# nicrie/xmca

Hardware: AMD Instinct MI355X
Metric: MCA solve+rotate throughput (ms_per_step = solve+rotate wall-clock, ms); rule_n surrogates/s in `rule_n` (higher is better)
Workload: dtype f64; 1 GPU; C2: synthetic EOF T=2920 x N=10000 float64 (generator A), solve() + rotate(n_rot=10, power=1); parallelism=replicas x1 (solve/rotate do not shard); rule_n run-sharded x1

## Files before the change

### xmca_amd/csrc/jacobi.h

```cpp
#pragma once
#include <algorithm>
#include <cmath>
#include <cstring>

#include "common.h"
#include "gemm.h"
#include "cholesky.h"
#include "tridiag.h"
#include "tridiag_vec.h"
#include "jacobi_kernels.h"

namespace xmca {

struct EvdInfo {
  int sweeps = 0;
  int tile = 0;
  int slots = 0;
  double last_off = 0.0;
  int lr_step = 0;
  double diag_spread = 0;
  int tridiag = 0;
  int n_eigvec = 0;
};

// ... 279 lines not shown
                          std::vector<double>& lam_host, double* lam_dev, double* Zr, double* Zi, int64_t ldz,
                          EvdInfo* info = nullptr, bool nearly_diagonal = false, int n_lead = -1, TrdLeadHook* lead_hook = nullptr) {
  const bool cplx = Ai != nullptr;
  const bool part = Zr && n_lead >= 0 && n_lead < n;
  if (part) XMCA_CHECK(n_lead >= 1, XMCA_ERR_INVALID, "hermitian_evd: n_lead must be at least 1 when vectors are wanted");
  DevBuf<double> full[2];
  double *Fr = Zr, *Fi = Zi;
  int64_t ldf = ldz;
  auto all_rows = [&] {
    if (!part || Fr != Zr) return;
    Fr = full[0].ensure((size_t)n * n);
    Fi = cplx ? full[1].ensure((size_t)n * n) : nullptr;
    ldf = n;
  };
  auto hand_out = [&] {
    if (!part) return;
    const size_t row = sizeof(double) * (size_t)n;
    XMCA_HIP(hipMemcpy2DAsync(Zr, sizeof(double) * (size_t)ldz, Fr, row, row, (size_t)n_lead, hipMemcpyDeviceToDevice, st));
    if (cplx) XMCA_HIP(hipMemcpy2DAsync(Zi, sizeof(double) * (size_t)ldz, Fi, row, row, (size_t)n_lead, hipMemcpyDeviceToDevice, st));
    XMCA_HIP(hipStreamSynchronize(st));
  };
  const int trd_min_n = [] { const char* e = std::getenv("XMCA_TRIDIAG_MIN_N"); return e ? std::atoi(e) : 192; }();
  if (!Zr && !nearly_diagonal && trd_enabled() && n >= trd_min_n && trd_fits(n, Ai != nullptr)) {
    TrdParams P = trd_reduce(st, ws.trd, Ar, Ai, n, lda, false);
    if (xmca_trace("trdsum")) trd_trace_checksums(st, P, Ar, n, lda);
    trd_eigenvalues(st, ws.trd, P, lam_host, lam_dev, ws.lam_tmp);
    if (info) {
      *info = EvdInfo{};
      info->tridiag = 1;
    }
    return;
  }
  if (Zr && !nearly_diagonal && evd_vectors_by_reduction(n, Ai != nullptr)) {
    ws.trdv.count_call();
    TrdParams P = trd_reduce(st, ws.trd, Ar, Ai, n, lda, true);
    trd_wy_prepare(st, ws.trdv, ws.gws, P, Ai != nullptr);
    std::vector<double> lam_t;
    trd_eigenvalues(st, ws.trd, P, lam_t, lam_dev, ws.lam_tmp, ws.trdv.lam_asc.ensure((size_t)n));
    if (part) {
      const int kp = trd_partial_count(lam_t, n, n_lead);
      bool ran = false, done = false;
      const bool rep_lead = trd_repeated_leading(lam_t, n, kp);
      if (kp < n && !rep_lead) {
        ran = true;
        done = trd_eigenvectors_partial(st, ws.trdv, ws.gws, P, cplx, kp, n_lead, Zr, Zi, ldz);
      }
      if (xmca_trace("solve"))
        std::fprintf(stderr, "xmca: eigh n = %d, %d leading vectors wanted: %d formed%s\n", n, n_lead, done ? kp : n,
                     done ? "" : (kp >= n ? " (no gap within the cap)" : rep_lead ? " (repeated eigenvalues)" : " (clean-up refused)"));
      if (done) {
        XMCA_HIP(hipStreamSynchronize(st));
        lam_host = lam_t;
        if (info) {
          *info = EvdInfo{};
          info->tridiag = 1;
          info->n_eigvec = kp;
        }
        return;
      }
      if (ran) ws.trdv.prepared = true;
    }
    bool repeated = false;
    {
      const double lmax = n > 0 ? std::max(std::fabs(lam_t.front()), std::fabs(lam_t.back())) : 0.0;
      for (int i = 0; i + 1 < n && !repeated; ++i) repeated = lam_t[(size_t)i] - lam_t[(size_t)i + 1] <= 2.2e-16 * lmax;
      if (repeated && xmca_trace("solve")) std::fprintf(stderr, "xmca: eigh n = %d: repeated eigenvalues - block Jacobi instead of twisted vectors\n", n);
    }
    if (repeated) {
      if (ws.trdv.prepared && !ws.trdv.joined && ws.trdv.side) XMCA_HIP(hipStreamSynchronize(ws.trdv.side));
      ws.trdv.prepared = false;
      ws.trdv.joined = true;
    }
    if (!repeated) all_rows();
    if (!repeated && trd_eigenvectors(st, ws.trd, ws.trdv, ws.gws, P, Ai != nullptr, Fr, Fi, ldf, part ? nullptr : lead_hook)) {
      XMCA_HIP(hipStreamSynchronize(st));
      lam_host = lam_t;
      if (info) {
        *info = EvdInfo{};
        info->tridiag = 1;
        info->n_eigvec = n;
      }
      hand_out();
      return;
    }
  }
  const double tol = Zr ? 1e-10 : 1e-8;
  all_rows();
  if (Ai) jacobi_evd<true, 32>(st, ws, Ar, Ai, n, lda, lam_host, lam_dev, Fr, Fi, ldf, tol, info);
  else if (n > 32) jacobi_evd<false, 64>(st, ws, Ar, nullptr, n, lda, lam_host, lam_dev, Fr, nullptr, ldf, tol, info);
  else jacobi_evd<false, 32>(st, ws, Ar, nullptr, n, lda, lam_host, lam_dev, Fr, nullptr, ldf, tol, info);
  hand_out();
}

}
// ... 1 lines not shown
```

### xmca_amd/csrc/tridiag.h

```cpp
#pragma once
#include <algorithm>
#include <cmath>
#include <cstring>
#include <vector>

#include "common.h"

namespace xmca {

constexpr int TRD_THREADS = 512;
constexpr int TRD_ROWS = 4;
constexpr int TRD_MAX_WGS = 256;
constexpr int TRD_MAX_ITERS = 32;

struct TrdParams {
  double* Ar;
  double* Ai;
  int64_t ld;
  int n;
  double* vb[2][2];
  double* pb[2][2];
  double* gp[2][2];
  double* tau[2];
  double* d;
  double* e;
  double* Vr;
// ... 900 lines not shown
    if (CPLX) { double* t1 = bV[1]; bV[1] = bX[1]; bX[1] = t1; }
    tpr = tr_next;
    tpi = ti_next;
    spr = sr_next;
    spi = si_next;
  }
}

__global__ void trd_prefill_kernel(const double* __restrict__ Wr, const double* __restrict__ Wi, int n, double* __restrict__ xch) {
  const int k = blockIdx.x * blockDim.x + threadIdx.x;
  if (k >= n) return;
  if (Wi) {
    xch[2 * k] = trd_untagged(Wr[k]);
    xch[2 * k + 1] = trd_untagged(Wi[k]);
  } else {
    xch[2 * k] = trd_untagged(Wr[k]);
  }
}

__global__ __launch_bounds__(256) void trd_maxabs_kernel(const double* __restrict__ Ar, const double* __restrict__ Ai, int n, int64_t lda,
                                                         unsigned long long* __restrict__ acc) {
  double m = 0.0;
  bool bad = false;
  for (int r = blockIdx.x; r < n; r += gridDim.x)
    for (int c = threadIdx.x; c < n; c += 256) {
      const double a = fabs(Ar[(int64_t)r * lda + c]), b = Ai ? fabs(Ai[(int64_t)r * lda + c]) : 0.0;
      if (!(a <= 1.7e308) || !(b <= 1.7e308)) bad = true;
      m = fmax(m, fmax(a, b));
    }
  for (int o = 32; o > 0; o >>= 1) m = fmax(m, __shfl_xor(m, o));
  if (__any(bad)) { if ((threadIdx.x & 63) == 0) atomicOr(acc + 1, 1ull); }
  else if ((threadIdx.x & 63) == 0 && m > 0.0) atomicMax(acc, (unsigned long long)__double_as_longlong(m));
}
__global__ void trd_scale_kernel(const unsigned long long* __restrict__ acc, double* __restrict__ scal) {
  const double g = __longlong_as_double((long long)acc[0]);
  const bool nan = acc[1] != 0ull;
  double f = 1.0;
  if (g > 0.0 && !nan) {
    int ex;
    frexp(g, &ex);
    f = ldexp(1.0, -ex);
  }
  scal[0] = f;
  scal[1] = nan ? 1.0 : 0.0;
}

__global__ void trd_copy_kernel(const double* __restrict__ Ar, const double* __restrict__ Ai, int n, int64_t lda, double* Wr, double* Wi,
                                int64_t ld, const double* __restrict__ scal) {
  const double f = scal[0];
  const int r = blockIdx.x;
  for (int c = threadIdx.x; c < ld; c += blockDim.x) {
    const bool in = c < n;
    Wr[(int64_t)r * ld + c] = in ? f * Ar[(int64_t)r * lda + c] : 0.0;
    if (Wi) Wi[(int64_t)r * ld + c] = in ? f * Ai[(int64_t)r * lda + c] : 0.0;
  }
}

constexpr int TRD_BIS_THREADS = 256;
__global__ __launch_bounds__(TRD_BIS_THREADS) void trd_bisect_kernel(const double* __restrict__ d, const double* __restrict__ e, int n,
                                                                   const double* __restrict__ scal, double* lam_desc, double* lam_asc_scaled, int* flag) {
  extern __shared__ __attribute__((aligned(16))) double bis_lds[];
  __shared__ double red[2][TRD_BIS_THREADS / 64];
  double* sd = bis_lds;
  double* se2 = bis_lds + n;
  const int tid = threadIdx.x;
  double gl = 1.7e308, gu = -1.7e308;
  bool bad = false;
// ... 74 lines not shown
  if (live && l == 0) {
    lam_desc[n - 1 - k] = 0.5 * (lo + hi) / scal[0];
    if (lam_asc_scaled) lam_asc_scaled[k] = 0.5 * (lo + hi);
  }
}

struct TrdWorkspace {
  DevBuf<double> W[2];
  DevBuf<double> V[2];
  DevBuf<double> vec;
  DevBuf<double> scal;
  DevBuf<int> flag;
  DevBuf<unsigned long long> prof;
  DevBuf<double> sync;
  DevBuf<unsigned int> flags;
  int resident_used = 0;
  int stages_used = 0;
  std::string last_desc;
  hipEvent_t ev[2] = {nullptr, nullptr};
  bool ev_pending = false;
  double reduce_ms = 0.0;
  long long reduce_calls = 0;
  long long resident_calls = 0;
  void ev_begin(hipStream_t st) {
    if (!ev[0]) { XMCA_HIP(hipEventCreate(&ev[0])); XMCA_HIP(hipEventCreate(&ev[1])); }
    XMCA_HIP(hipEventRecord(ev[0], st));
  }
  void ev_end(hipStream_t st) { XMCA_HIP(hipEventRecord(ev[1], st)); ev_pending = true; }
  void ev_collect() {
    if (!ev_pending) return;
    float t = 0.f;
    if (hipEventSynchronize(ev[1]) == hipSuccess && hipEventElapsedTime(&t, ev[0], ev[1]) == hipSuccess) { reduce_ms += t; ++reduce_calls; }
    ev_pending = false;
  }
  ~TrdWorkspace() { if (ev[0]) { (void)hipEventDestroy(ev[0]); (void)hipEventDestroy(ev[1]); } }
  double ms = 0.0;
};

inline bool trd_enabled() {
  const char* e = std::getenv("XMCA_TRIDIAG");
  return !(e && e[0] == '0');
}

inline size_t trd_step_lds(int n, bool cplx) { return (size_t)(((n + 3) + 1) & ~1) * 3 * (cplx ? 2 : 1) * sizeof(double); }

inline bool trd_fits(int n, bool cplx) {
// ... 84 lines not shown
      for (int cnc = nc - 4; cnc >= 4; cnc -= 4) {
        const int cap = cnc * 128;
        if (n <= cap) continue;
        const int c = ((n - cap + 255) / 256) * 256;
        if (c < n - 256 && (cuts.empty() || c > cuts.back())) cuts.push_back(c);
      }
    }
  }
  int begin = 0;
  for (size_t q = 0; q <= cuts.size(); ++q) {
    const int end = q < cuts.size() ? cuts[q] : n;
    TrdStage sg{};
    sg.col0 = begin;
    sg.nc = (q == 0 && !chain) ? nc : trd_stage_nc(n - begin, cplx);
    sg.rr = (q > 0 && chain && trd_pack_lanes()) ? trd_stage_rr_packed(sg.nc, cplx) : trd_stage_rr(sg.nc, cplx);
    sg.j_begin = begin;
    sg.j_end = end;
    st.push_back(sg);
    begin = end;
  }
  return st;
}

inline TrdParams trd_reduce(hipStream_t st, TrdWorkspace& ws, const double* Ar, const double* Ai, int n, int64_t lda, bool keep_reflectors) {
  const bool cplx = Ai != nullptr;
  const int nc = trd_resident_nc(n, cplx);
  const std::vector<TrdStage> stages = trd_plan(n, cplx, nc);
  int64_t ld = std::max<int64_t>(((int64_t)n + 2 + 15) & ~(int64_t)15, (int64_t)nc * 128);
  for (const TrdStage& sg : stages) ld = std::max<int64_t>(ld, (int64_t)sg.col0 + (int64_t)sg.nc * 128);
  const size_t nv = (size_t)((n + 8 + 15) & ~15);
  ws.W[0].ensure((size_t)n * ld);
  if (cplx) ws.W[1].ensure((size_t)n * ld);
  if (keep_reflectors) {
    ws.V[0].ensure((size_t)n * ld);
    XMCA_HIP(hipMemsetAsync(ws.V[0].get(), 0, sizeof(double) * (size_t)n * ld, st));
    if (cplx) {
      ws.V[1].ensure((size_t)n * ld);
      XMCA_HIP(hipMemsetAsync(ws.V[1].get(), 0, sizeof(double) * (size_t)n * ld, st));
    }
  }
  ws.vec.ensure(TrdLayout::doubles(nv));
  ws.scal.ensure(4);
  ws.flag.ensure(4);
  XMCA_HIP(hipMemsetAsync(ws.vec.get(), 0, sizeof(double) * TrdLayout::doubles(nv), st));
  XMCA_HIP(hipMemsetAsync(ws.flag.get(), 0, sizeof(int) * 4, st));
  TrdLayout lay{n, ld, nv, ws.vec.get()};
  TrdParams P = lay.params(ws.W[0].get(), cplx ? ws.W[1].get() : nullptr, keep_reflectors ? ws.V[0].get() : nullptr,
                           (keep_reflectors && cplx) ? ws.V[1].get() : nullptr);
  {
    unsigned long long* acc = reinterpret_cast<unsigned long long*>(ws.scal.get() + 2);
    XMCA_HIP(hipMemsetAsync(acc, 0, 2 * sizeof(unsigned long long), st));
    hipLaunchKernelGGL(trd_maxabs_kernel, dim3(std::min(n, 1024)), dim3(256), 0, st, Ar, Ai, n, lda, acc);
    hipLaunchKernelGGL(trd_scale_kernel, dim3(1), dim3(1), 0, st, acc, ws.scal.get());
  }
  hipLaunchKernelGGL(trd_copy_kernel, dim3(n), dim3(256), 0, st, Ar, Ai, n, lda, P.Ar, P.Ai, ld, ws.scal.get());
  ws.resident_used = 0;

  if (nc > 0) {
    PersistGate& gate = persist_gate();
    const int n_cus = gate.n_cus;
    const size_t lv = (size_t)(ld > (int64_t)nc * 128 ? ld : (int64_t)nc * 128);
    const size_t rec = cplx ? 4 : 2;
    const size_t sync_doubles = 2 * lv + 8 + 2 * rec * lv;
    ws.sync.ensure(sync_doubles);
    ws.flags.ensure(4);
    XMCA_HIP(hipMemsetAsync(ws.sync.get(), 0, sizeof(double) * sync_doubles, st));
    XMCA_HIP(hipMemsetAsync(ws.flags.get(), 0, sizeof(unsigned int) * 4, st));
    TrdSync S{};
    double* q = ws.sync.get();
    for (int c = 0; c < 2; ++c) { S.hand_u[c] = q; q += lv; }
    S.hand_s = q; q += 8;
    S.xch = q;
    S.xch_pb = (int)(rec * lv * sizeof(double));
    S.contiguous = in_surrogate_lanes() ? 1 : 0;
    S.spin_limit = trd_spin_limit();
    hipLaunchKernelGGL(trd_prefill_kernel, dim3(ceil_div(n, 256)), dim3(256), 0, st, P.Ar, P.Ai, n, S.xch);
    S.give_up = reinterpret_cast<int*>(ws.flags.get());
    using ResFn = void (*)(TrdParams, TrdSync, int);
    auto pick = [&](int snc, int srr) -> ResFn {
      if (cplx) {
        switch (snc) {
          case 4: return srr == 2 ? trd_resident_kernel<true, 4, 2> : trd_resident_kernel<true, 4, 1>;
          case 8: return srr == 2 ? trd_resident_kernel<true, 8, 2> : trd_resident_kernel<true, 8, 1>;
          case 12: return srr == 3 ? trd_resident_kernel<true, 12, 3> : trd_resident_kernel<true, 12, 2>;
          case 16: return trd_resident_kernel<true, 16, 2>;
          default: return trd_resident_kernel<true, 20, 2>;
        }
      }
      switch (snc) {
        case 4: return trd_resident_kernel<false, 4, 1>;
        case 8: return trd_resident_kernel<false, 8, 1>;
        case 12: return trd_resident_kernel<false, 12, 2>;
        case 16: return trd_resident_kernel<false, 16, 2>;
        case 20: return trd_resident_kernel<false, 20, 3>;
        default: return trd_resident_kernel<false, 24, 3>;
      }
    };
    static const char* prof_file_r = std::getenv("XMCA_TRD_PROF");
    if (prof_file_r) {
      P.prof = ws.prof.ensure((size_t)8 * n);
      XMCA_HIP(hipMemsetAsync(P.prof, 0, sizeof(unsigned long long) * 8 * (size_t)n, st));
    }
    int gave_up = 0;
    {
      PersistGate::Claim claim(gate, n_cus);
      ws.ev_begin(st);
      for (size_t q = 0; q < stages.size(); ++q) {
        const TrdStage& sg = stages[q];
        const int c0 = sg.col0, ns = n - c0;
        const int64_t off = (int64_t)c0 * ld + c0;
        TrdParams Pq = P;
        Pq.n = ns;
        Pq.Ar = P.Ar + off;
        if (P.Ai) Pq.Ai = P.Ai + off;
        Pq.d = P.d + c0; Pq.e = P.e + c0;
        Pq.tau[0] = P.tau[0] + c0; Pq.tau[1] = P.tau[1] + c0;
        if (P.Vr) Pq.Vr = P.Vr + off;
        if (P.Vi) Pq.Vi = P.Vi + off;
        if (P.prof) Pq.prof = P.prof + (size_t)8 * c0;
        TrdSync Sq = S;
        Sq.hand_u[0] = S.hand_u[0] + c0; Sq.hand_u[1] = S.hand_u[1] + c0;
        Sq.xch = S.xch + 2 * (size_t)c0;
        Sq.j_begin = sg.j_begin - c0;
        Sq.j_end = sg.j_end - c0;
        Sq.cont = q > 0 ? 1 : 0;
        const int wgs = std::max(1, std::min(std::min(n_cus, TRD_MAX_WGS), ceil_div(ns, (TRD_RES_THREADS / 64) * sg.rr)));
        const int first_res = std::max(0, ns - wgs * (TRD_RES_THREADS / 64) * sg.rr);
        const size_t lds = (size_t)sg.nc * 128 * 3 * (cplx ? 2 : 1) * sizeof(double);
        ResFn fn = pick(sg.nc, sg.rr);
        XMCA_HIP(hipFuncSetAttribute(reinterpret_cast<const void*>(fn), hipFuncAttributeMaxDynamicSharedMemorySize, 150 * 1024));
        hipLaunchKernelGGL(fn, dim3(wgs), dim3(TRD_RES_THREADS), lds, st, Pq, Sq, first_res);
      }
      ws.ev_end(st);
      XMCA_HIP(hipGetLastError());
      int dbg[4] = {0};
      XMCA_HIP(hipMemcpyAsync(dbg, S.give_up, sizeof(dbg), hipMemcpyDeviceToHost, st));
      XMCA_HIP(hipStreamSynchronize(st));
      gave_up = dbg[0];
      if (gave_up && xmca_trace("giveup"))
        std::fprintf(stderr, "xmca: trd_resident_kernel: workgroup %d ran out of its spins at column %d of its launch (n = %d, %d launches)\n", dbg[3], dbg[2], n, (int)stages.size());
    }
    ws.stages_used = (int)stages.size();
    {
      std::string d = stages.size() > 1 ? "chain of " + std::to_string(stages.size()) + " persistent launches: " : "";
      for (size_t q = 0; q < stages.size(); ++q) {
        const TrdStage& sg = stages[q];
        d += (q ? " -> " : "") + std::string("trd_resident_kernel<") + (cplx ? "complex" : "real") + ",NC=" + std::to_string(sg.nc) + ",RR=" + std::to_string(sg.rr) +
             ",tagged> columns [" + std::to_string(sg.j_begin) + "," + std::to_string(sg.j_end) + ")";
      }
      ws.last_desc = d;
    }
    if (prof_file_r) {
      std::vector<unsigned long long> hp((size_t)8 * n);
      XMCA_HIP(hipMemcpy(hp.data(), P.prof, sizeof(unsigned long long) * hp.size(), hipMemcpyDeviceToHost));
      if (FILE* f = std::fopen(prof_file_r, "w")) {
        for (int j = 0; j < n; ++j) {
          for (int q = 0; q < 7; ++q) std::fprintf(f, "%llu ", hp[(size_t)8 * j + q] - (q ? hp[(size_t)8 * j] : (j ? hp[(size_t)8 * (j - 1)] : hp[0])));
          std::fprintf(f, "\n");
        }
        std::fclose(f);
      }
      P.prof = nullptr;
    }
    if (!gave_up) {
      ws.resident_used = 1;
      ++ws.resident_calls;
      ws.ev_collect();
      return P;
    }
    ws.ev_pending = false;
    ws.resident_used = 2;
    ++persist_giveups();
    if (xmca_trace("giveup")) std::fprintf(stderr, "xmca: trd_resident_kernel (n = %d) gave up - repeated with one launch per column\n", n);
    hipLaunchKernelGGL(trd_copy_kernel, dim3(n), dim3(256), 0, st, Ar, Ai, n, lda, P.Ar, P.Ai, ld, ws.scal.get());
    XMCA_HIP(hipMemsetAsync(ws.vec.get(), 0, sizeof(double) * TrdLayout::doubles(nv), st));
    if (keep_reflectors) {
      XMCA_HIP(hipMemsetAsync(ws.V[0].get(), 0, sizeof(double) * (size_t)n * ld, st));
      if (cplx) XMCA_HIP(hipMemsetAsync(ws.V[1].get(), 0, sizeof(double) * (size_t)n * ld, st));
    }
  }

  ws.last_desc = std::string("trd_step_kernel<") + (cplx ? "complex" : "real") + "> x " + std::to_string(n) + " launches (one per column)";
  const size_t lds = trd_step_lds(n, cplx);
  const int slots = ((n + 3) + 1) & ~1;
  const int ns = slots <= 2 * TRD_THREADS ? 2 : slots <= 4 * TRD_THREADS ? 4 : slots <= 8 * TRD_THREADS ? 8 : 16;
  using StepFn = void (*)(TrdParams, int, int);
  StepFn fn = nullptr;
  XMCA_CHECK(!cplx || ns <= 8, XMCA_ERR_UNSUPPORTED, "trd_reduce: complex problem too large for the LDS of a workgroup");
  if (cplx) fn = ns == 2 ? trd_step_kernel<true, 2> : ns == 4 ? trd_step_kernel<true, 4> : trd_step_kernel<true, 8>;
  else fn = ns == 2 ? trd_step_kernel<false, 2> : ns == 4 ? trd_step_kernel<false, 4> : ns == 8 ? trd_step_kernel<false, 8> : trd_step_kernel<false, 16>;
  XMCA_HIP(hipFuncSetAttribute(reinterpret_cast<const void*>(fn), hipFuncAttributeMaxDynamicSharedMemorySize, 150 * 1024));
  static const char* prof_file = std::getenv("XMCA_TRD_PROF");
  if (prof_file) {
    P.prof = ws.prof.ensure((size_t)8 * n);
    XMCA_HIP(hipMemsetAsync(P.prof, 0, sizeof(unsigned long long) * 8 * (size_t)n, st));
  }
  int wgs_prev = 1;
  ws.ev_begin(st);
  for (int j = 0; j < n; ++j) {
    const int m = n - j - 1;
    const int wgs = std::max(1, std::min(TRD_MAX_WGS, (m + TRD_ROWS - 1) / TRD_ROWS));
    hipLaunchKernelGGL(fn, dim3(wgs), dim3(TRD_THREADS), lds, st, P, j, wgs_prev);
    wgs_prev = wgs;
  }
  ws.ev_end(st);
  XMCA_HIP(hipGetLastError());
  if (prof_file) {
    std::vector<unsigned long long> hp((size_t)8 * n);
    XMCA_HIP(hipMemcpyAsync(hp.data(), P.prof, sizeof(unsigned long long) * hp.size(), hipMemcpyDeviceToHost, st));
    XMCA_HIP(hipStreamSynchronize(st));
    if (FILE* f = std::fopen(prof_file, "w")) {
      for (int j = 0; j < n; ++j) {
        for (int q = 0; q < 7; ++q) std::fprintf(f, "%llu ", hp[(size_t)8 * j + q] - (q ? hp[(size_t)8 * j] : 0ull));
        std::fprintf(f, "\n");
      }
      std::fclose(f);
    }
  }
  return P;
}

inline void trd_trace_checksums(hipStream_t st, const TrdParams& P, const double* Ar, int n, int64_t lda) {
  std::vector<double> in((size_t)n * lda), d(n), e(n);
  XMCA_HIP(hipStreamSynchronize(st));
  XMCA_HIP(hipMemcpy(in.data(), Ar, sizeof(double) * in.size(), hipMemcpyDeviceToHost));
  XMCA_HIP(hipMemcpy(d.data(), P.d, sizeof(double) * n, hipMemcpyDeviceToHost));
  XMCA_HIP(hipMemcpy(e.data(), P.e, sizeof(double) * n, hipMemcpyDeviceToHost));
  unsigned long long ci = 1469598103934665603ull, co = ci;
  for (int i = 0; i < n; ++i) for (int j = 0; j < n; ++j) { unsigned long long b; std::memcpy(&b, &in[(size_t)i * lda + j], 8); ci = (ci ^ b) * 1099511628211ull; }
  for (int i = 0; i < n; ++i) { unsigned long long b; std::memcpy(&b, &d[i], 8); co = (co ^ b) * 1099511628211ull; if (i + 1 < n) { std::memcpy(&b, &e[i], 8); co = (co ^ b) * 1099511628211ull; } }
  std::fprintf(stderr, "trdsum n=%d in=%016llx out=%016llx\n", n, ci, co);
  if (const char* dir = std::getenv("XMCA_TRD_DUMP_DIR")) {
    char name[512];
    std::snprintf(name, sizeof(name), "%s/de_%016llx_%016llx.bin", dir, ci, co);
    if (FILE* f0 = std::fopen(name, "rb")) std::fclose(f0);
    else if (FILE* f1 = std::fopen(name, "wb")) { std::fwrite(d.data(), 8, n, f1); std::fwrite(e.data(), 8, n, f1); std::fclose(f1); }
  }
}

inline void trd_eigenvalues(hipStream_t st, TrdWorkspace& ws, const TrdParams& P, std::vector<double>& lam_host, double* lam_dev,
                            DevBuf<double>& lam_tmp, double* lam_asc_scaled = nullptr) {
  const int n = P.n;
  double* out = lam_dev ? lam_dev : lam_tmp.ensure((size_t)n);
  XMCA_HIP(hipFuncSetAttribute(reinterpret_cast<const void*>(trd_bisect_kernel), hipFuncAttributeMaxDynamicSharedMemorySize, 150 * 1024));
  hipLaunchKernelGGL(trd_bisect_kernel, dim3(ceil_div(n, TRD_BIS_THREADS / 16)), dim3(TRD_BIS_THREADS), sizeof(double) * 2 * (size_t)n, st, P.d,
                     P.e, n, ws.scal.get(), out, lam_asc_scaled, ws.flag.get());
  XMCA_HIP(hipGetLastError());
  lam_host.resize((size_t)n);
  int flag = 0;
  double scal[2] = {1.0, 0.0};
  XMCA_HIP(hipMemcpyAsync(lam_host.data(), out, sizeof(double) * n, hipMemcpyDeviceToHost, st));
  XMCA_HIP(hipMemcpyAsync(&flag, ws.flag.get(), sizeof(int), hipMemcpyDeviceToHost, st));
  XMCA_HIP(hipMemcpyAsync(scal, ws.scal.get(), sizeof(double) * 2, hipMemcpyDeviceToHost, st));
  XMCA_HIP(hipStreamSynchronize(st));
  ws.ev_collect();
  XMCA_CHECK(flag == 0 && scal[1] == 0.0, XMCA_ERR_NUMERIC, "SVD failed. NaN entries may be the problem.");
}

}
```

### xmca_amd/csrc/tridiag_vec.h

```cpp
#pragma once
#include "cholesky.h"
#include "tridiag.h"

namespace xmca {

__device__ __forceinline__ double trd_lane_value(double v, int u) {
  const int lo = __builtin_amdgcn_readlane(__double2loint(v), u), hi = __builtin_amdgcn_readlane(__double2hiint(v), u);
  return __hiloint2double(hi, lo);
}

__global__ __launch_bounds__(128) void trd_twisted_kernel(const double* __restrict__ d, const double* __restrict__ e, int n, int nev,
                                                         const double* __restrict__ lam, double* __restrict__ W, double* __restrict__ Yt,
                                                         int64_t ldy) {
  __shared__ double nrm_sh[2][64];
  __shared__ int idx_sh[2][64];
  const int lane = threadIdx.x & 63, half = threadIdx.x >> 6;
  const int k = blockIdx.x * 64 + lane;
  const bool live = k < nev;
  const int kk = live ? k : nev - 1;
  const double l = lam[kk];
  if (n == 1) { if (live && half == 0) Yt[k] = 1.0; return; }
  constexpr int B = 32;
  double emax = 0.0;
  for (int i = lane; i < n - 1; i += 64) emax = fmax(emax, fabs(e[i]));
// ... 282 lines not shown
      for (int s = 0; s < nsb; ++s)
        for (int a = Q * s; a < Q * s + Q / 2; ++a)
          for (int b = Q * s + Q / 2; b < std::min(Q * s + Q, nt); ++b)
            add(a, b, 128 * (Q * s + (lv == 0 ? Q / 2 : 0)), 128 * (Q * s + (lv == 0 ? Q : Q / 2)));
      done(lv == 0 ? lev_p[2] : lev_t[2]);
    }
    for (int bm = 0; bm < nt; ++bm) {
      const int s = bm / Q;
      for (int bn = Q * s; bn < nt; ++bn) add(bm, bn, 128 * bm, std::min(128 * (Q * s + Q), n));
    }
    done(tv);
  }
};

struct TrdVecWorkspace {
  DevBuf<double> Y[2];
  DevBuf<double> Wk[2];
  DevBuf<double> S[2];
  DevBuf<double> small;
  DevBuf<double> band[2];
  DevBuf<double> TV[2];
  TrdBackPlan plan;
  hipStream_t side = nullptr;
  hipEvent_t ev_fork = nullptr, ev_join = nullptr;
  GemmWorkspace side_gws;
  bool prepared = false, joined = true;
  int calls = 0;
  void count_call() {
    if (side || in_surrogate_lanes() || ++calls < 2) return;
    PersistGate& gate = persist_gate();
    PersistGate::Claim alone(gate, gate.n_cus);
    side_init();
  }
  void side_init() {
    if (side) return;
    XMCA_HIP(hipStreamCreateWithFlags(&side, hipStreamNonBlocking));
    XMCA_HIP(hipEventCreateWithFlags(&ev_fork, hipEventDisableTiming));
    XMCA_HIP(hipEventCreateWithFlags(&ev_join, hipEventDisableTiming));
  }
  ~TrdVecWorkspace() {
    if (side) {
      (void)hipStreamSynchronize(side);
      (void)hipEventDestroy(ev_fork);
      (void)hipEventDestroy(ev_join);
      (void)hipStreamDestroy(side);
    }
  }
  TrdVecWorkspace() = default;
  TrdVecWorkspace(const TrdVecWorkspace&) = delete;
  TrdVecWorkspace& operator=(const TrdVecWorkspace&) = delete;
  DevBuf<double> lam_asc;
  DevBuf<double> lead, lead_part;
  DevBuf<unsigned long long> orth;
  double last_orth = 0.0;
  int ns_steps = 0;
};

inline void trd_wy_prepare(hipStream_t st, TrdVecWorkspace& vw, GemmWorkspace& gws_main, const TrdParams& P, bool cplx) {
  const int n = P.n;
  const int64_t ldv = P.ld;
  constexpr int SBK = TRD_SBK;
  const int nref = n - 1;
  if (vw.prepared && vw.side) XMCA_HIP(hipStreamSynchronize(vw.side));
  vw.prepared = false;
  if (nref <= 0) return;
  if (vw.plan.n != n) vw.plan.build(st, n);
  const bool use_side = vw.side != nullptr && !in_surrogate_lanes();
  PoolScope scope(use_side ? nullptr : current_pool());
  if (use_side) {
    XMCA_HIP(hipEventRecord(vw.ev_fork, st));
    XMCA_HIP(hipStreamWaitEvent(vw.side, vw.ev_fork, 0));
  }
  {
    hipStream_t st_main = st;
    hipStream_t st = use_side ? vw.side : st_main;
    GemmWorkspace& gws = use_side ? vw.side_gws : gws_main;
    const TrdBackPlan& pl = vw.plan;
    const int nsb = ceil_div(n, SBK), npad = nsb * SBK;
    const size_t bsz = (size_t)nsb * ((size_t)SBK * SBK + SBK) + SBK;
    double* bnd[2] = {vw.band[0].ensure(3 * bsz), cplx ? vw.band[1].ensure(3 * bsz) : nullptr};
    for (int c = 0; c < (cplx ? 2 : 1); ++c) XMCA_HIP(hipMemsetAsync(bnd[c], 0, sizeof(double) * 3 * bsz, st));
    double *Sr_ = bnd[0], *Tr_ = bnd[0] + bsz, *Pr_ = bnd[0] + 2 * bsz;
    double *Si_ = cplx ? bnd[1] : nullptr, *Ti_ = cplx ? bnd[1] + bsz : nullptr, *Pi_ = cplx ? bnd[1] + 2 * bsz : nullptr;
    cgemm<double>(st, gws, P.Vr, P.Vi, ldv, true, true, P.Vr, P.Vi, ldv, false, false, Sr_, Si_, SBK, n, n, n, 1.0, nullptr, nullptr, false,
                  0.0, &pl.gram);
    if (cplx) hipLaunchKernelGGL(trd_wy_tinv_kernel<true>, dim3(ceil_div(n, 64)), dim3(64), 0, st, Sr_, Si_, Tr_, Ti_, (int64_t)SBK, nref, P.tau[0], P.tau[1]);
    else hipLaunchKernelGGL(trd_wy_tinv_kernel<false>, dim3(ceil_div(n, 64)), dim3(64), 0, st, Sr_, nullptr, Tr_, nullptr, (int64_t)SBK, nref, P.tau[0], nullptr);
// ... 11 lines not shown
  if (use_side) XMCA_HIP(hipEventRecord(vw.ev_join, vw.side));
  vw.joined = !use_side;
  vw.prepared = true;
}

struct TrdCleanupProduct {
  const double *Cr = nullptr, *Ci = nullptr, *Yr = nullptr, *Yi = nullptr;
  int64_t ld = 0;
  double *Zr = nullptr, *Zi = nullptr;
  int64_t ldz = 0;
  int n = 0;
};
inline void trd_cleanup_product(hipStream_t st, GemmWorkspace& gws, const TrdCleanupProduct& p) {
  cgemm<double>(st, gws, p.Cr, p.Ci, p.ld, true, false, p.Yr, p.Yi, p.ld, false, true, p.Zr, p.Zi, p.ldz, p.n, p.n, p.n, 1.0, nullptr, nullptr, false);
}
struct TrdLeadHook {
  int rows = 0;
  bool defer = false;
  const double* lead = nullptr;
  bool pending = false;
  TrdCleanupProduct product;
};

inline bool trd_eigenvectors(hipStream_t st, TrdWorkspace& ws, TrdVecWorkspace& vw, GemmWorkspace& gws, const TrdParams& P, bool cplx,
                             double* Zr, double* Zi, int64_t ldz, TrdLeadHook* hook = nullptr) {
  const int n = P.n;
  const int64_t ldv = P.ld;
  constexpr int SBK = TRD_SBK;
  const int64_t ld = ((int64_t)n + 15) & ~(int64_t)15;
  const size_t plane = (size_t)n * ld;
  double* Yr = vw.Y[0].ensure(plane);
  double* Yi = cplx ? vw.Y[1].ensure(plane) : nullptr;
  double* Wr = vw.Wk[0].ensure(plane);
  double* Wi = cplx ? vw.Wk[1].ensure(plane) : nullptr;
  hipLaunchKernelGGL(trd_twisted_kernel, dim3(ceil_div(n, 64)), dim3(128), 0, st, P.d, P.e, n, n, vw.lam_asc.get(), Wr, Yr, ld);
  XMCA_HIP(hipGetLastError());
  if (cplx) XMCA_HIP(hipMemsetAsync(Yi, 0, sizeof(double) * plane, st));
  const int nref = n - 1;
  if (nref > 0) {
    XMCA_CHECK(vw.prepared, XMCA_ERR_STATE, "trd_eigenvectors: trd_wy_prepare has not run");
    vw.prepared = false;
    if (!vw.joined) XMCA_HIP(hipStreamWaitEvent(st, vw.ev_join, 0));
    vw.joined = true;
    const double* TVr = vw.TV[0].get();
    const double* TVi = cplx ? vw.TV[1].get() : nullptr;
    double* sm = vw.small.ensure(2 * (size_t)SBK * ld);
    double* Xr = sm; double* Xi = cplx ? Xr + (size_t)SBK * ld : nullptr;
    for (int j0 = ((nref - 1) / SBK) * SBK; j0 >= 0; j0 -= SBK) {
      const int nb = std::min(SBK, nref - j0);
      const int i0 = j0 + 1, mb = n - i0;
      const int64_t vo = (int64_t)j0 * ldv + i0;
      double* Zr0 = Yr + (int64_t)i0 * ld;
      double* Zi0 = cplx ? Yi + (int64_t)i0 * ld : nullptr;
      cgemm<double>(st, gws, TVr + vo, cplx ? TVi + vo : nullptr, ldv, true, false, Zr0, Zi0, ld, true, false, Xr, Xi, ld, nb, n, mb, 1.0, nullptr,
                    nullptr, false);
      cgemm<double>(st, gws, P.Vr + vo, cplx ? P.Vi + vo : nullptr, ldv, false, false, Xr, Xi, ld, true, false, Zr0, Zi0, ld, mb, n, nb, -1.0,
                    nullptr, nullptr, false, 1.0);
    }
  }
  XMCA_HIP(hipGetLastError());
  double* Sr = vw.S[0].ensure(plane);
  double* Si = cplx ? vw.S[1].ensure(plane) : nullptr;
  vw.orth.ensure(2);
  vw.ns_steps = 0;
  for (int round = 0; round < 3; ++round) {
    cgemm<double>(st, gws, Yr, Yi, ld, false, true, Yr, Yi, ld, true, false, Sr, Si, ld, n, n, n, 1.0, nullptr, nullptr, true);
// ... 109 lines not shown
```

Baseline: 37.79 solve+rotate/s.

## Defer resident-kernel give-up check and overlap twisted vectors with eigenvalue readback

The host synchronisation after the persistent tridiagonal reduction is dropped. Its give-up status is now read together with the eigenvalue readback, and if it gave up the reduction is repeated with per-column launches. When vectors are wanted, the WY preparation and twisted eigenvector kernel are queued behind the bisection, while the host copies run on the side stream so the GPU keeps working during the readback. Several memsets are merged into one zeroing kernel, and maxabs is unrolled with a per-workgroup reduction before the atomics. The cost is more complex state handling, with a guard to abandon pending late work and a retry path on give-up.

Result: no change. 38.08 solve+rotate/s (median of 6 runs) (+0.8%).

```diff
diff --git a/xmca_amd/csrc/jacobi.h b/xmca_amd/csrc/jacobi.h
--- a/xmca_amd/csrc/jacobi.h
+++ b/xmca_amd/csrc/jacobi.h
@@ -325,9 +325,14 @@
   };
   const int trd_min_n = [] { const char* e = std::getenv("XMCA_TRIDIAG_MIN_N"); return e ? std::atoi(e) : 192; }();
   if (!Zr && !nearly_diagonal && trd_enabled() && n >= trd_min_n && trd_fits(n, Ai != nullptr)) {
-    TrdParams P = trd_reduce(st, ws.trd, Ar, Ai, n, lda, false);
-    if (xmca_trace("trdsum")) trd_trace_checksums(st, P, Ar, n, lda);
-    trd_eigenvalues(st, ws.trd, P, lam_host, lam_dev, ws.lam_tmp);
+    const bool trdsum = xmca_trace("trdsum");
+    TrdLateGuard late_guard{st, ws.trd};
+    TrdParams P = trd_reduce(st, ws.trd, Ar, Ai, n, lda, false, !trdsum && !in_surrogate_lanes());
+    if (trdsum) trd_trace_checksums(st, P, Ar, n, lda);
+    if (!trd_eigenvalues(st, ws.trd, P, lam_host, lam_dev, ws.lam_tmp)) {
+      P = trd_reduce_repeat(st, ws.trd, P, Ar, Ai, n, lda, false);
+      trd_eigenvalues(st, ws.trd, P, lam_host, lam_dev, ws.lam_tmp);
+    }
     if (info) {
       *info = EvdInfo{};
       info->tridiag = 1;
@@ -336,10 +341,26 @@
   }
   if (Zr && !nearly_diagonal && evd_vectors_by_reduction(n, Ai != nullptr)) {
     ws.trdv.count_call();
-    TrdParams P = trd_reduce(st, ws.trd, Ar, Ai, n, lda, true);
-    trd_wy_prepare(st, ws.trdv, ws.gws, P, Ai != nullptr);
+    TrdLateGuard late_guard{st, ws.trd};
+    TrdParams P = trd_reduce(st, ws.trd, Ar, Ai, n, lda, true, !in_surrogate_lanes());
     std::vector<double> lam_t;
-    trd_eigenvalues(st, ws.trd, P, lam_t, lam_dev, ws.lam_tmp, ws.trdv.lam_asc.ensure((size_t)n));
+    auto eigenvalues = [&] {
+      trd_wy_prepare(st, ws.trdv, ws.gws, P, cplx);
+      double* lam_asc = ws.trdv.lam_asc.ensure((size_t)n);
+      const bool ahead = !part && ws.trdv.side && ws.trdv.prepared && !ws.trdv.joined;
+      if (!ahead) return trd_eigenvalues(st, ws.trd, P, lam_t, lam_dev, ws.lam_tmp, lam_asc);
+      return trd_eigenvalues(st, ws.trd, P, lam_t, lam_dev, ws.lam_tmp, lam_asc, [&] { trd_twisted_queue(st, ws.trdv, P, cplx); },
+                             ws.trdv.side, ws.trdv.ev_read);
+    };
+    if (!eigenvalues()) {
+      XMCA_HIP(hipStreamSynchronize(st));
+      if (ws.trdv.side) XMCA_HIP(hipStreamSynchronize(ws.trdv.side));
+      ws.trdv.prepared = false;
+      ws.trdv.joined = true;
+      ws.trdv.twisted_queued = false;
+      P = trd_reduce_repeat(st, ws.trd, P, Ar, Ai, n, lda, true);
+      eigenvalues();
+    }
     if (part) {
       const int kp = trd_partial_count(lam_t, n, n_lead);
       bool ran = false, done = false;
@@ -373,6 +394,7 @@
       if (ws.trdv.prepared && !ws.trdv.joined && ws.trdv.side) XMCA_HIP(hipStreamSynchronize(ws.trdv.side));
       ws.trdv.prepared = false;
       ws.trdv.joined = true;
+      ws.trdv.twisted_queued = false;
     }
     if (!repeated) all_rows();
     if (!repeated && trd_eigenvectors(st, ws.trd, ws.trdv, ws.gws, P, Ai != nullptr, Fr, Fi, ldf, part ? nullptr : lead_hook)) {
diff --git a/xmca_amd/csrc/tridiag.h b/xmca_amd/csrc/tridiag.h
--- a/xmca_amd/csrc/tridiag.h
+++ b/xmca_amd/csrc/tridiag.h
@@ -2,6 +2,7 @@
 #include <algorithm>
 #include <cmath>
 #include <cstring>
+#include <memory>
 #include <vector>
 
 #include "common.h"
@@ -948,15 +949,42 @@
                                                          unsigned long long* __restrict__ acc) {
   double m = 0.0;
   bool bad = false;
-  for (int r = blockIdx.x; r < n; r += gridDim.x)
-    for (int c = threadIdx.x; c < n; c += 256) {
-      const double a = fabs(Ar[(int64_t)r * lda + c]), b = Ai ? fabs(Ai[(int64_t)r * lda + c]) : 0.0;
+  constexpr int U = 4;
+  for (int r = blockIdx.x; r < n; r += gridDim.x) {
+    const double* ar = Ar + (int64_t)r * lda;
+    const double* ai = Ai ? Ai + (int64_t)r * lda : nullptr;
+    int c = threadIdx.x;
+    for (; c + (U - 1) * 256 < n; c += U * 256) {
+      double a[U], b[U];
+#pragma unroll
+      for (int u = 0; u < U; ++u) a[u] = fabs(ar[c + u * 256]);
+#pragma unroll
+      for (int u = 0; u < U; ++u) b[u] = ai ? fabs(ai[c + u * 256]) : 0.0;
+#pragma unroll
+      for (int u = 0; u < U; ++u) {
+        if (!(a[u] <= 1.7e308) || !(b[u] <= 1.7e308)) bad = true;
+        m = fmax(m, fmax(a[u], b[u]));
+      }
+    }
+    for (; c < n; c += 256) {
+      const double a = fabs(ar[c]), b = ai ? fabs(ai[c]) : 0.0;
       if (!(a <= 1.7e308) || !(b <= 1.7e308)) bad = true;
       m = fmax(m, fmax(a, b));
     }
+  }
   for (int o = 32; o > 0; o >>= 1) m = fmax(m, __shfl_xor(m, o));
-  if (__any(bad)) { if ((threadIdx.x & 63) == 0) atomicOr(acc + 1, 1ull); }
-  else if ((threadIdx.x & 63) == 0 && m > 0.0) atomicMax(acc, (unsigned long long)__double_as_longlong(m));
+  __shared__ double m_sh[4];
+  __shared__ int bad_sh[4];
+  const int wave = threadIdx.x >> 6;
+  const int wave_bad = __any(bad) ? 1 : 0;
+  if ((threadIdx.x & 63) == 0) { m_sh[wave] = m; bad_sh[wave] = wave_bad; }
+  __syncthreads();
+  if (threadIdx.x == 0) {
+    const bool any_bad = (bad_sh[0] | bad_sh[1] | bad_sh[2] | bad_sh[3]) != 0;
+    m = fmax(fmax(m_sh[0], m_sh[1]), fmax(m_sh[2], m_sh[3]));
+    if (any_bad) atomicOr(acc + 1, 1ull);
+    else if (m > 0.0) atomicMax(acc, (unsigned long long)__double_as_longlong(m));
+  }
 }
 __global__ void trd_scale_kernel(const unsigned long long* __restrict__ acc, double* __restrict__ scal) {
   const double g = __longlong_as_double((long long)acc[0]);
@@ -969,6 +997,17 @@
   }
   scal[0] = f;
   scal[1] = nan ? 1.0 : 0.0;
+}
+
+struct TrdZero {
+  void* p[5];
+  size_t words[5];
+};
+__global__ __launch_bounds__(256) void trd_zero_kernel(TrdZero z) {
+  for (int q = 0; q < 5; ++q) {
+    unsigned int* p = static_cast<unsigned int*>(z.p[q]);
+    for (size_t i = (size_t)blockIdx.x * 256 + threadIdx.x; i < z.words[q]; i += (size_t)gridDim.x * 256) p[i] = 0u;
+  }
 }
 
 __global__ void trd_copy_kernel(const double* __restrict__ Ar, const double* __restrict__ Ai, int n, int64_t lda, double* Wr, double* Wi,
@@ -1089,6 +1128,9 @@
   double reduce_ms = 0.0;
   long long reduce_calls = 0;
   long long resident_calls = 0;
+  bool late_pending = false;
+  int late_dbg[4] = {0, 0, 0, 0};
+  std::unique_ptr<PersistGate::Claim> late_claim;
   void ev_begin(hipStream_t st) {
     if (!ev[0]) { XMCA_HIP(hipEventCreate(&ev[0])); XMCA_HIP(hipEventCreate(&ev[1])); }
     XMCA_HIP(hipEventRecord(ev[0], st));
@@ -1219,7 +1261,98 @@
   return st;
 }
 
-inline TrdParams trd_reduce(hipStream_t st, TrdWorkspace& ws, const double* Ar, const double* Ai, int n, int64_t lda, bool keep_reflectors) {
+inline TrdParams trd_reduce_columns(hipStream_t st, TrdWorkspace& ws, TrdParams P, const double* Ar, const double* Ai, int n, int64_t lda,
+                                    bool keep_reflectors, bool repeat) {
+  const bool cplx = Ai != nullptr;
+  if (repeat) {
+    const int64_t ld = P.ld;
+    const size_t nv = (size_t)((n + 8 + 15) & ~15);
+    ws.ev_pending = false;
+    ws.resident_used = 2;
+    ++persist_giveups();
+    if (xmca_trace("giveup")) std::fprintf(stderr, "xmca: trd_resident_kernel (n = %d) gave up - repeated with one launch per column\n", n);
+    hipLaunchKernelGGL(trd_copy_kernel, dim3(n), dim3(256), 0, st, Ar, Ai, n, lda, P.Ar, P.Ai, ld, ws.scal.get());
+    XMCA_HIP(hipMemsetAsync(ws.vec.get(), 0, sizeof(double) * TrdLayout::doubles(nv), st));
+    if (keep_reflectors) {
+      XMCA_HIP(hipMemsetAsync(ws.V[0].get(), 0, sizeof(double) * (size_t)n * ld, st));
+      if (cplx) XMCA_HIP(hipMemsetAsync(ws.V[1].get(), 0, sizeof(double) * (size_t)n * ld, st));
+    }
+  }
+
+  ws.last_desc = std::string("trd_step_kernel<") + (cplx ? "complex" : "real") + "> x " + std::to_string(n) + " launches (one per column)";
+  const size_t lds = trd_step_lds(n, cplx);
+  const int slots = ((n + 3) + 1) & ~1;
+  const int ns = slots <= 2 * TRD_THREADS ? 2 : slots <= 4 * TRD_THREADS ? 4 : slots <= 8 * TRD_THREADS ? 8 : 16;
+  using StepFn = void (*)(TrdParams, int, int);
+  StepFn fn = nullptr;
+  XMCA_CHECK(!cplx || ns <= 8, XMCA_ERR_UNSUPPORTED, "trd_reduce: complex problem too large for the LDS of a workgroup");
+  if (cplx) fn = ns == 2 ? trd_step_kernel<true, 2> : ns == 4 ? trd_step_kernel<true, 4> : trd_step_kernel<true, 8>;
+  else fn = ns == 2 ? trd_step_kernel<false, 2> : ns == 4 ? trd_step_kernel<false, 4> : ns == 8 ? trd_step_kernel<false, 8> : trd_step_kernel<false, 16>;
+  XMCA_HIP(hipFuncSetAttribute(reinterpret_cast<const void*>(fn), hipFuncAttributeMaxDynamicSharedMemorySize, 150 * 1024));
+  static const char* prof_file = std::getenv("XMCA_TRD_PROF");
+  if (prof_file) {
+    P.prof = ws.prof.ensure((size_t)8 * n);
+    XMCA_HIP(hipMemsetAsync(P.prof, 0, sizeof(unsigned long long) * 8 * (size_t)n, st));
+  }
+  int wgs_prev = 1;
+  ws.ev_begin(st);
+  for (int j = 0; j < n; ++j) {
+    const int m = n - j - 1;
+    const int wgs = std::max(1, std::min(TRD_MAX_WGS, (m + TRD_ROWS - 1) / TRD_ROWS));
+    hipLaunchKernelGGL(fn, dim3(wgs), dim3(TRD_THREADS), lds, st, P, j, wgs_prev);
+    wgs_prev = wgs;
+  }
+  ws.ev_end(st);
+  XMCA_HIP(hipGetLastError());
+  if (prof_file) {
+    std::vector<unsigned long long> hp((size_t)8 * n);
+    XMCA_HIP(hipMemcpyAsync(hp.data(), P.prof, sizeof(unsigned long long) * hp.size(), hipMemcpyDeviceToHost, st));
+    XMCA_HIP(hipStreamSynchronize(st));
+    if (FILE* f = std::fopen(prof_file, "w")) {
+      for (int j = 0; j < n; ++j) {
+        for (int q = 0; q < 7; ++q) std::fprintf(f, "%llu ", hp[(size_t)8 * j + q] - (q ? hp[(size_t)8 * j] : 0ull));
+        std::fprintf(f, "\n");
+      }
+      std::fclose(f);
+    }
+  }
+  return P;
+}
+
+inline bool trd_gave_up(TrdWorkspace& ws, int n) {
+  const char* e = std::getenv("XMCA_TRD_FORCE_GIVEUP");
+  const bool gave_up = ws.late_dbg[0] != 0 || (e && e[0] == '1');
+  if (gave_up && ws.late_dbg[0] && xmca_trace("giveup"))
+    std::fprintf(stderr, "xmca: trd_resident_kernel: workgroup %d ran out of its spins at column %d of its launch (n = %d, %d launches)\n",
+                 ws.late_dbg[3], ws.late_dbg[2], n, ws.stages_used);
+  return gave_up;
+}
+inline bool trd_reduce_settle(TrdWorkspace& ws, int n) {
+  if (!ws.late_pending) return true;
+  ws.late_pending = false;
+  ws.late_claim.reset();
+  if (trd_gave_up(ws, n)) return false;
+  ws.resident_used = 1;
+  ++ws.resident_calls;
+  ws.ev_collect();
+  return true;
+}
+inline TrdParams trd_reduce_repeat(hipStream_t st, TrdWorkspace& ws, const TrdParams& P, const double* Ar, const double* Ai, int n, int64_t lda,
+                                   bool keep_reflectors) {
+  XMCA_HIP(hipMemsetAsync(ws.flag.get(), 0, sizeof(int) * 4, st));
+  return trd_reduce_columns(st, ws, P, Ar, Ai, n, lda, keep_reflectors, true);
+}
+inline void trd_late_abandon(hipStream_t st, TrdWorkspace& ws) {
+  if (!ws.late_pending) return;
+  (void)hipStreamSynchronize(st);
+  ws.late_pending = false;
+  ws.ev_pending = false;
+  ws.late_claim.reset();
+}
+
+inline TrdParams trd_reduce(hipStream_t st, TrdWorkspace& ws, const double* Ar, const double* Ai, int n, int64_t lda, bool keep_reflectors,
+                            bool late = false) {
+  trd_late_abandon(st, ws);
   const bool cplx = Ai != nullptr;
   const int nc = trd_resident_nc(n, cplx);
   const std::vector<TrdStage> stages = trd_plan(n, cplx, nc);
@@ -1239,14 +1372,25 @@
   ws.vec.ensure(TrdLayout::doubles(nv));
   ws.scal.ensure(4);
   ws.flag.ensure(4);
-  XMCA_HIP(hipMemsetAsync(ws.vec.get(), 0, sizeof(double) * TrdLayout::doubles(nv), st));
-  XMCA_HIP(hipMemsetAsync(ws.flag.get(), 0, sizeof(int) * 4, st));
+  const size_t lv = (size_t)(ld > (int64_t)nc * 128 ? ld : (int64_t)nc * 128);
+  const size_t rec = cplx ? 4 : 2;
+  const size_t sync_doubles = 2 * lv + 8 + 2 * rec * lv;
+  {
+    TrdZero z{};
+    z.p[0] = ws.vec.get(); z.words[0] = TrdLayout::doubles(nv) * 2;
+    z.p[1] = ws.flag.get(); z.words[1] = 4;
+    z.p[2] = ws.scal.get() + 2; z.words[2] = 4;
+    if (nc > 0) {
+      z.p[3] = ws.sync.ensure(sync_doubles); z.words[3] = sync_doubles * 2;
+      z.p[4] = ws.flags.ensure(4); z.words[4] = 4;
+    }
+    hipLaunchKernelGGL(trd_zero_kernel, dim3(64), dim3(256), 0, st, z);
+  }
   TrdLayout lay{n, ld, nv, ws.vec.get()};
   TrdParams P = lay.params(ws.W[0].get(), cplx ? ws.W[1].get() : nullptr, keep_reflectors ? ws.V[0].get() : nullptr,
                            (keep_reflectors && cplx) ? ws.V[1].get() : nullptr);
   {
     unsigned long long* acc = reinterpret_cast<unsigned long long*>(ws.scal.get() + 2);
-    XMCA_HIP(hipMemsetAsync(acc, 0, 2 * sizeof(unsigned long long), st));
     hipLaunchKernelGGL(trd_maxabs_kernel, dim3(std::min(n, 1024)), dim3(256), 0, st, Ar, Ai, n, lda, acc);
     hipLaunchKernelGGL(trd_scale_kernel, dim3(1), dim3(1), 0, st, acc, ws.scal.get());
   }
@@ -1256,13 +1400,6 @@
   if (nc > 0) {
     PersistGate& gate = persist_gate();
     const int n_cus = gate.n_cus;
-    const size_t lv = (size_t)(ld > (int64_t)nc * 128 ? ld : (int64_t)nc * 128);
-    const size_t rec = cplx ? 4 : 2;
-    const size_t sync_doubles = 2 * lv + 8 + 2 * rec * lv;
-    ws.sync.ensure(sync_doubles);
-    ws.flags.ensure(4);
-    XMCA_HIP(hipMemsetAsync(ws.sync.get(), 0, sizeof(double) * sync_doubles, st));
-    XMCA_HIP(hipMemsetAsync(ws.flags.get(), 0, sizeof(unsigned int) * 4, st));
     TrdSync S{};
     double* q = ws.sync.get();
     for (int c = 0; c < 2; ++c) { S.hand_u[c] = q; q += lv; }
@@ -1298,9 +1435,18 @@
       P.prof = ws.prof.ensure((size_t)8 * n);
       XMCA_HIP(hipMemsetAsync(P.prof, 0, sizeof(unsigned long long) * 8 * (size_t)n, st));
     }
+    auto describe = [&] {
+      std::string d = stages.size() > 1 ? "chain of " + std::to_string(stages.size()) + " persistent launches: " : "";
+      for (size_t q = 0; q < stages.size(); ++q) {
+        const TrdStage& sg = stages[q];
+        d += (q ? " -> " : "") + std::string("trd_resident_kernel<") + (cplx ? "complex" : "real") + ",NC=" + std::to_string(sg.nc) + ",RR=" + std::to_string(sg.rr) +
+             ",tagged> columns [" + std::to_string(sg.j_begin) + "," + std::to_string(sg.j_end) + ")";
+      }
+      ws.last_desc = d;
+    };
     int gave_up = 0;
     {
-      PersistGate::Claim claim(gate, n_cus);
+      auto claim = std::make_unique<PersistGate::Claim>(gate, n_cus);
       ws.ev_begin(st);
       for (size_t q = 0; q < stages.size(); ++q) {
         const TrdStage& sg = stages[q];
@@ -1330,22 +1476,17 @@
       }
       ws.ev_end(st);
       XMCA_HIP(hipGetLastError());
-      int dbg[4] = {0};
-      XMCA_HIP(hipMemcpyAsync(dbg, S.give_up, sizeof(dbg), hipMemcpyDeviceToHost, st));
+      ws.stages_used = (int)stages.size();
+      describe();
+      if (late && !prof_file_r) {
+        ws.late_claim = std::move(claim);
+        ws.late_pending = true;
+        ws.resident_used = 1;
+        return P;
+      }
+      XMCA_HIP(hipMemcpyAsync(ws.late_dbg, S.give_up, sizeof(ws.late_dbg), hipMemcpyDeviceToHost, st));
       XMCA_HIP(hipStreamSynchronize(st));
-      gave_up = dbg[0];
-      if (gave_up && xmca_trace("giveup"))
-        std::fprintf(stderr, "xmca: trd_resident_kernel: workgroup %d ran out of its spins at column %d of its launch (n = %d, %d launches)\n", dbg[3], dbg[2], n, (int)stages.size());
-    }
-    ws.stages_used = (int)stages.size();
-    {
-      std::string d = stages.size() > 1 ? "chain of " + std::to_string(stages.size()) + " persistent launches: " : "";
-      for (size_t q = 0; q < stages.size(); ++q) {
-        const TrdStage& sg = stages[q];
-        d += (q ? " -> " : "") + std::string("trd_resident_kernel<") + (cplx ? "complex" : "real") + ",NC=" + std::to_string(sg.nc) + ",RR=" + std::to_string(sg.rr) +
-             ",tagged> columns [" + std::to_string(sg.j_begin) + "," + std::to_string(sg.j_end) + ")";
-      }
-      ws.last_desc = d;
+      gave_up = trd_gave_up(ws, n);
     }
     if (prof_file_r) {
       std::vector<unsigned long long> hp((size_t)8 * n);
@@ -1365,56 +1506,9 @@
       ws.ev_collect();
       return P;
     }
-    ws.ev_pending = false;
-    ws.resident_used = 2;
-    ++persist_giveups();
-    if (xmca_trace("giveup")) std::fprintf(stderr, "xmca: trd_resident_kernel (n = %d) gave up - repeated with one launch per column\n", n);
-    hipLaunchKernelGGL(trd_copy_kernel, dim3(n), dim3(256), 0, st, Ar, Ai, n, lda, P.Ar, P.Ai, ld, ws.scal.get());
-    XMCA_HIP(hipMemsetAsync(ws.vec.get(), 0, sizeof(double) * TrdLayout::doubles(nv), st));
-    if (keep_reflectors) {
-      XMCA_HIP(hipMemsetAsync(ws.V[0].get(), 0, sizeof(double) * (size_t)n * ld, st));
-      if (cplx) XMCA_HIP(hipMemsetAsync(ws.V[1].get(), 0, sizeof(double) * (size_t)n * ld, st));
-    }
-  }
-
-  ws.last_desc = std::string("trd_step_kernel<") + (cplx ? "complex" : "real") + "> x " + std::to_string(n) + " launches (one per column)";
-  const size_t lds = trd_step_lds(n, cplx);
-  const int slots = ((n + 3) + 1) & ~1;
-  const int ns = slots <= 2 * TRD_THREADS ? 2 : slots <= 4 * TRD_THREADS ? 4 : slots <= 8 * TRD_THREADS ? 8 : 16;
-  using StepFn = void (*)(TrdParams, int, int);
-  StepFn fn = nullptr;
-  XMCA_CHECK(!cplx || ns <= 8, XMCA_ERR_UNSUPPORTED, "trd_reduce: complex problem too large for the LDS of a workgroup");
-  if (cplx) fn = ns == 2 ? trd_step_kernel<true, 2> : ns == 4 ? trd_step_kernel<true, 4> : trd_step_kernel<true, 8>;
-  else fn = ns == 2 ? trd_step_kernel<false, 2> : ns == 4 ? trd_step_kernel<false, 4> : ns == 8 ? trd_step_kernel<false, 8> : trd_step_kernel<false, 16>;
-  XMCA_HIP(hipFuncSetAttribute(reinterpret_cast<const void*>(fn), hipFuncAttributeMaxDynamicSharedMemorySize, 150 * 1024));
-  static const char* prof_file = std::getenv("XMCA_TRD_PROF");
-  if (prof_file) {
-    P.prof = ws.prof.ensure((size_t)8 * n);
-    XMCA_HIP(hipMemsetAsync(P.prof, 0, sizeof(unsigned long long) * 8 * (size_t)n, st));
-  }
-  int wgs_prev = 1;
-  ws.ev_begin(st);
-  for (int j = 0; j < n; ++j) {
-    const int m = n - j - 1;
-    const int wgs = std::max(1, std::min(TRD_MAX_WGS, (m + TRD_ROWS - 1) / TRD_ROWS));
-    hipLaunchKernelGGL(fn, dim3(wgs), dim3(TRD_THREADS), lds, st, P, j, wgs_prev);
-    wgs_prev = wgs;
-  }
-  ws.ev_end(st);
-  XMCA_HIP(hipGetLastError());
-  if (prof_file) {
-    std::vector<unsigned long long> hp((size_t)8 * n);
-    XMCA_HIP(hipMemcpyAsync(hp.data(), P.prof, sizeof(unsigned long long) * hp.size(), hipMemcpyDeviceToHost, st));
-    XMCA_HIP(hipStreamSynchronize(st));
-    if (FILE* f = std::fopen(prof_file, "w")) {
-      for (int j = 0; j < n; ++j) {
-        for (int q = 0; q < 7; ++q) std::fprintf(f, "%llu ", hp[(size_t)8 * j + q] - (q ? hp[(size_t)8 * j] : 0ull));
-        std::fprintf(f, "\n");
-      }
-      std::fclose(f);
-    }
-  }
-  return P;
+    return trd_reduce_columns(st, ws, P, Ar, Ai, n, lda, keep_reflectors, true);
+  }
+  return trd_reduce_columns(st, ws, P, Ar, Ai, n, lda, keep_reflectors, false);
 }
 
 inline void trd_trace_checksums(hipStream_t st, const TrdParams& P, const double* Ar, int n, int64_t lda) {
@@ -1435,23 +1529,41 @@
   }
 }
 
-inline void trd_eigenvalues(hipStream_t st, TrdWorkspace& ws, const TrdParams& P, std::vector<double>& lam_host, double* lam_dev,
-                            DevBuf<double>& lam_tmp, double* lam_asc_scaled = nullptr) {
+struct TrdLateGuard {
+  hipStream_t st;
+  TrdWorkspace& ws;
+  ~TrdLateGuard() { trd_late_abandon(st, ws); }
+};
+struct TrdQueueNothing { void operator()() const {} };
+template <typename QueueBehind = TrdQueueNothing>
+inline bool trd_eigenvalues(hipStream_t st, TrdWorkspace& ws, const TrdParams& P, std::vector<double>& lam_host, double* lam_dev,
+                            DevBuf<double>& lam_tmp, double* lam_asc_scaled = nullptr, QueueBehind&& queue_behind = QueueBehind(),
+                            hipStream_t rd = nullptr, hipEvent_t ev_rd = nullptr) {
   const int n = P.n;
   double* out = lam_dev ? lam_dev : lam_tmp.ensure((size_t)n);
   XMCA_HIP(hipFuncSetAttribute(reinterpret_cast<const void*>(trd_bisect_kernel), hipFuncAttributeMaxDynamicSharedMemorySize, 150 * 1024));
   hipLaunchKernelGGL(trd_bisect_kernel, dim3(ceil_div(n, TRD_BIS_THREADS / 16)), dim3(TRD_BIS_THREADS), sizeof(double) * 2 * (size_t)n, st, P.d,
                      P.e, n, ws.scal.get(), out, lam_asc_scaled, ws.flag.get());
   XMCA_HIP(hipGetLastError());
+  hipStream_t cp = st;
+  if (rd && ev_rd) {
+    XMCA_HIP(hipEventRecord(ev_rd, st));
+    queue_behind();
+    XMCA_HIP(hipStreamWaitEvent(rd, ev_rd, 0));
+    cp = rd;
+  }
   lam_host.resize((size_t)n);
   int flag = 0;
   double scal[2] = {1.0, 0.0};
-  XMCA_HIP(hipMemcpyAsync(lam_host.data(), out, sizeof(double) * n, hipMemcpyDeviceToHost, st));
-  XMCA_HIP(hipMemcpyAsync(&flag, ws.flag.get(), sizeof(int), hipMemcpyDeviceToHost, st));
-  XMCA_HIP(hipMemcpyAsync(scal, ws.scal.get(), sizeof(double) * 2, hipMemcpyDeviceToHost, st));
-  XMCA_HIP(hipStreamSynchronize(st));
+  if (ws.late_pending) XMCA_HIP(hipMemcpyAsync(ws.late_dbg, ws.flags.get(), sizeof(ws.late_dbg), hipMemcpyDeviceToHost, cp));
+  XMCA_HIP(hipMemcpyAsync(lam_host.data(), out, sizeof(double) * n, hipMemcpyDeviceToHost, cp));
+  XMCA_HIP(hipMemcpyAsync(&flag, ws.flag.get(), sizeof(int), hipMemcpyDeviceToHost, cp));
+  XMCA_HIP(hipMemcpyAsync(scal, ws.scal.get(), sizeof(double) * 2, hipMemcpyDeviceToHost, cp));
+  XMCA_HIP(hipStreamSynchronize(cp));
+  if (!trd_reduce_settle(ws, n)) return false;
   ws.ev_collect();
   XMCA_CHECK(flag == 0 && scal[1] == 0.0, XMCA_ERR_NUMERIC, "SVD failed. NaN entries may be the problem.");
-}
-
-}
+  return true;
+}
+
+}
diff --git a/xmca_amd/csrc/tridiag_vec.h b/xmca_amd/csrc/tridiag_vec.h
--- a/xmca_amd/csrc/tridiag_vec.h
+++ b/xmca_amd/csrc/tridiag_vec.h
@@ -328,9 +328,10 @@
   DevBuf<double> TV[2];
   TrdBackPlan plan;
   hipStream_t side = nullptr;
-  hipEvent_t ev_fork = nullptr, ev_join = nullptr;
+  hipEvent_t ev_fork = nullptr, ev_join = nullptr, ev_read = nullptr;
   GemmWorkspace side_gws;
   bool prepared = false, joined = true;
+  bool twisted_queued = false;
   int calls = 0;
   void count_call() {
     if (side || in_surrogate_lanes() || ++calls < 2) return;
@@ -343,12 +344,14 @@
     XMCA_HIP(hipStreamCreateWithFlags(&side, hipStreamNonBlocking));
     XMCA_HIP(hipEventCreateWithFlags(&ev_fork, hipEventDisableTiming));
     XMCA_HIP(hipEventCreateWithFlags(&ev_join, hipEventDisableTiming));
+    XMCA_HIP(hipEventCreateWithFlags(&ev_read, hipEventDisableTiming));
   }
   ~TrdVecWorkspace() {
     if (side) {
       (void)hipStreamSynchronize(side);
       (void)hipEventDestroy(ev_fork);
       (void)hipEventDestroy(ev_join);
+      (void)hipEventDestroy(ev_read);
       (void)hipStreamDestroy(side);
     }
   }
@@ -369,6 +372,7 @@
   const int nref = n - 1;
   if (vw.prepared && vw.side) XMCA_HIP(hipStreamSynchronize(vw.side));
   vw.prepared = false;
+  vw.twisted_queued = false;
   if (nref <= 0) return;
   if (vw.plan.n != n) vw.plan.build(st, n);
   const bool use_side = vw.side != nullptr && !in_surrogate_lanes();
@@ -426,6 +430,26 @@
   TrdCleanupProduct product;
 };
 
+inline void trd_twisted_queue(hipStream_t st, TrdVecWorkspace& vw, const TrdParams& P, bool cplx) {
+  const int n = P.n;
+  const int64_t ld = ((int64_t)n + 15) & ~(int64_t)15;
+  const size_t plane = (size_t)n * ld;
+  double* Yr = vw.Y[0].ensure(plane);
+  double* Yi = cplx ? vw.Y[1].ensure(plane) : nullptr;
+  double* Wr = vw.Wk[0].ensure(plane);
+  if (cplx) vw.Wk[1].ensure(plane);
+  hipLaunchKernelGGL(trd_twisted_kernel, dim3(ceil_div(n, 64)), dim3(128), 0, st, P.d, P.e, n, n, vw.lam_asc.get(), Wr, Yr, ld);
+  XMCA_HIP(hipGetLastError());
+  if (cplx) XMCA_HIP(hipMemsetAsync(Yi, 0, sizeof(double) * plane, st));
+  if (n - 1 > 0) {
+    XMCA_CHECK(vw.prepared, XMCA_ERR_STATE, "trd_eigenvectors: trd_wy_prepare has not run");
+    vw.prepared = false;
+    if (!vw.joined) XMCA_HIP(hipStreamWaitEvent(st, vw.ev_join, 0));
+    vw.joined = true;
+  }
+  vw.twisted_queued = true;
+}
+
 inline bool trd_eigenvectors(hipStream_t st, TrdWorkspace& ws, TrdVecWorkspace& vw, GemmWorkspace& gws, const TrdParams& P, bool cplx,
                              double* Zr, double* Zi, int64_t ldz, TrdLeadHook* hook = nullptr) {
   const int n = P.n;
@@ -433,19 +457,14 @@
   constexpr int SBK = TRD_SBK;
   const int64_t ld = ((int64_t)n + 15) & ~(int64_t)15;
   const size_t plane = (size_t)n * ld;
-  double* Yr = vw.Y[0].ensure(plane);
-  double* Yi = cplx ? vw.Y[1].ensure(plane) : nullptr;
-  double* Wr = vw.Wk[0].ensure(plane);
-  double* Wi = cplx ? vw.Wk[1].ensure(plane) : nullptr;
-  hipLaunchKernelGGL(trd_twisted_kernel, dim3(ceil_div(n, 64)), dim3(128), 0, st, P.d, P.e, n, n, vw.lam_asc.get(), Wr, Yr, ld);
-  XMCA_HIP(hipGetLastError());
-  if (cplx) XMCA_HIP(hipMemsetAsync(Yi, 0, sizeof(double) * plane, st));
+  if (!vw.twisted_queued) trd_twisted_queue(st, vw, P, cplx);
+  vw.twisted_queued = false;
+  double* Yr = vw.Y[0].get();
+  double* Yi = cplx ? vw.Y[1].get() : nullptr;
+  double* Wr = vw.Wk[0].get();
+  double* Wi = cplx ? vw.Wk[1].get() : nullptr;
   const int nref = n - 1;
   if (nref > 0) {
-    XMCA_CHECK(vw.prepared, XMCA_ERR_STATE, "trd_eigenvectors: trd_wy_prepare has not run");
-    vw.prepared = false;
-    if (!vw.joined) XMCA_HIP(hipStreamWaitEvent(st, vw.ev_join, 0));
-    vw.joined = true;
     const double* TVr = vw.TV[0].get();
     const double* TVi = cplx ? vw.TV[1].get() : nullptr;
     double* sm = vw.small.ensure(2 * (size_t)SBK * ld);
```
